# mbed92/soft-grip

Measured on AMD Instinct MI355X. Metric: env steps/sec (whole node) at batch=4096, higher is better.
Workload: dtype f64; 1 GPU; configs[2]: 4096 envs/GPU, softbox scene (nv=118), stiffness ~ U(300,1400), reference 200-step squeeze schedule from reset, 7 substeps per env step; 327 equality rows (composite neighbour equalities on: DESIGN.md 2, U2); volume tendon damper integrated explicitly; envs_per_gpu=4096, envs_flagged_bad=0

## Files before the change

### include/softgrip.h

```cpp
#ifndef SOFTGRIP_H
#define SOFTGRIP_H

#include <stddef.h>
#include <stdint.h>

#ifdef __cplusplus
extern "C" {
#endif

typedef struct sg_model sg_model;
typedef struct sg_batch sg_batch;

typedef enum sg_status {
  SG_OK = 0,
  SG_ERR_INVALID = -1,
  SG_ERR_MODEL = -2,
  SG_ERR_NO_DEVICE = -3,
  SG_ERR_HIP = -4,
  SG_ERR_NOMEM = -5
} sg_status;

enum {
  SG_FLAG_BADQPOS = 1, SG_FLAG_BADQVEL = 2, SG_FLAG_BADQACC = 4,
  SG_FLAG_CONTACTFULL = 8, SG_FLAG_CNSTRFULL = 16, SG_FLAG_UNSUPPORTED_PAIR = 32
// ... 37 lines not shown

int sg_get_state(sg_batch* b, double* qpos, double* qvel, double* act, double* qacc_warmstart, double* ctrl, void* stream);
int sg_set_state(sg_batch* b, const double* qpos, const double* qvel, const double* act, const double* qacc_warmstart,
                 const double* ctrl, void* stream);

int sg_get_solver_stats(sg_batch* b, int32_t* ncon, int32_t* nefc, int32_t* iters, void* stream);

int sg_set_pipeline(sg_batch* b, int pipeline);

int sg_get_touch_words(sg_batch* b, int32_t* out, int nwords, void* stream);
int sg_model_nboxes(const sg_model* m);

int sg_set_solver_envs_per_wavefront(sg_batch* b, int epw);
int sg_solver_envs_per_wavefront(const sg_batch* b);

int sg_tree_workgroups_per_cu(const sg_batch* b);

int sg_get_poses(sg_batch* b, const int32_t* env_ids, int n_ids, double* xpos, double* xquat, double* geom_xpos, double* geom_xmat, void* stream);
int sg_model_nbody(const sg_model* m);
int sg_model_ngeom(const sg_model* m);

int sg_model_default_camera(const sg_model* m, double cam[7]);
int sg_render(sg_batch* b, const double* cam, const int32_t* env_ids, int n_ids, int width, int height,
              uint8_t* rgba, float* depth, int32_t* segid, void* stream);

int sg_model_set_skin(sg_model* m, int nvert, const int32_t* vert_body, const double* vert_pos,
                      int nface, const int32_t* face, const float rgba[4]);
int sg_model_skin(const sg_model* m, int* nvert, int* nface, int32_t* vert_body, double* vert_pos,
                  int32_t* face, float* rgba);

// ... 17 lines not shown
```

### soft-grip_amd/build_native.py

```python
import concurrent.futures
import contextlib
import sys
import fcntl
import glob
import hashlib
import os
import shutil
import subprocess
import tempfile

_HERE = os.path.dirname(os.path.abspath(__file__))
if _HERE not in sys.path:
    sys.path.insert(0, _HERE)
CSRC = os.path.join(_HERE, "csrc")
LIB = os.path.join(_HERE, "libsoftgrip.so")
LEGACY_LIB = os.path.join(_HERE, "libsoftgrip_legacy.so")
SOURCES = ["sg_api.hip", "sg_phase.hip", "sg_rows.hip", "sg_tree.hip", "sg_plan.cpp", "sg_mjcf.cpp"]
LEGACY_SOURCES = ["sg_legacy.hip"]
FLAGS = ["--offload-arch=gfx950", "-O3", "-std=c++17", "-fPIC", "-mllvm", "-amdgpu-sched-strategy=iterative-ilp"]
SOURCE_FLAGS = {"sg_tree.hip": ["-fno-optimize-sibling-calls"]}


def _headers():
    return sorted(glob.glob(os.path.join(CSRC, "*.h")) + glob.glob(os.path.join(CSRC, "*.inc")) + glob.glob(os.path.join(_HERE, "..", "include", "*.h")) + [os.path.join(CSRC, "sg_kernels.hip"), os.path.join(CSRC, "sg_kin.hip"), os.path.join(CSRC, "sg_contacts.hip"), os.path.abspath(__file__)])


def _stale(target, deps):
    if not os.path.exists(target):
        return True
    t = os.path.getmtime(target)
    return any(os.path.getmtime(d) > t for d in deps)


def needs_build(lib=LIB, sources=SOURCES):
    return _stale(lib, [os.path.join(CSRC, s) for s in sources] + _headers())
# ... 128 lines not shown
```

### soft-grip_amd/csrc/sg_api.hip

```cpp
#include <hip/hip_runtime.h>

#include <cstdio>
#include <cstring>
#include <memory>
#include <string>
#include <vector>

#include "sg_mjcf.h"
#include "sg_tree.h"
#include "sg_work.h"
#include "sg_kin.hip"
#include "sg_contacts.hip"
#include "sg_devmem.h"
#ifdef SG_LEGACY_PIPELINES
#include "sg_kernels_args.h"
#endif

#ifdef SG_LEGACY_PIPELINES
#define SG_LEGACY_ON 1
#else
#define SG_LEGACY_ON 0
#endif

namespace {
// ... 56 lines not shown
struct sg_batch {
  const sg_model* m = nullptr;
  int n = 0, device = 0;
  SgArena mem;
  SgArena tree_mem;
  SgPlanHeader* dH = nullptr;
  double *delem = nullptr, *qpos = nullptr, *qvel = nullptr, *warm = nullptr, *act = nullptr, *ctrl = nullptr, *kenv = nullptr, *ctrl_row = nullptr;
  SgGenPair* dgpairs = nullptr;
  int* dnbtab = nullptr;
  SgEqSlot* dsched = nullptr;
  unsigned* dtab = nullptr;
  int* dcpos = nullptr;
  int *kmask_jnt = nullptr, *kmask_ten = nullptr, *flags = nullptr, *touch = nullptr, *ncon = nullptr, *nefc = nullptr, *iters = nullptr;
  std::vector<int> kmask_jnt_host, kmask_ten_host;
  int epw_override = 0;
  int pipeline = 3;
  SgTreeBufs t;
  bool tree_ready = false;
  bool tree_attr_set = false;
  SgWork w = {};
  bool lds_attr_set = false;
  bool prof = false;
  std::vector<std::pair<hipEvent_t, hipEvent_t>> ev;
  double prof_ms = 0;
  long long prof_n = 0;
  std::vector<std::pair<hipEvent_t, hipEvent_t>> ev_pgs;
  std::vector<hipEvent_t> ev_pool;
  double prof_pgs_ms = 0;
  long long prof_pgs_n = 0;
  double* kin_d = nullptr;
// ... 314 lines not shown
  list.clear();
  if (avg_ms) *avg_ms = count ? sum_ms / count : 0.0;
  if (launches) *launches = count;
  if (reset) { sum_ms = 0; count = 0; }
  return SG_OK;
}

#define SG_EPW8_MIN_WAVES 1024
static int solver_epw(const sg_batch* b) {
  if (b->m->plan.h.nnb > 0) return 4;
  if (b->epw_override) return b->epw_override;
  if (const char* pe = getenv("SG_PGS_EPW")) return atoi(pe) == 4 ? 4 : 8;
  return (b->n + 7) / 8 >= SG_EPW8_MIN_WAVES ? 8 : 4;
}

static int launch_split(sg_batch* b, int mode, const uint8_t* mask, int nsub, double* sens, long long stride, int32_t* flags, int32_t* touch,
                        hipStream_t s) {
  const SgPlanHeader& H = b->m->plan.h;
  SgPhaseArgs pa;
  pa.H = b->dH; pa.elem = b->delem;
  pa.qpos = b->qpos; pa.qvel = b->qvel; pa.warm = b->warm; pa.act = b->act; pa.ctrl = b->ctrl;
  pa.kenv = b->kenv; pa.kmask_jnt = b->kmask_jnt; pa.kmask_ten = b->kmask_ten;
  pa.mask = mask; pa.sens = nullptr; pa.sens_stride = stride > 0 ? stride : H.nsensordata;
  pa.w = b->w; pa.nenv = b->n; pa.rowlayout = b->pipeline == 2;
  pa.nbtab = b->dnbtab; pa.cpos = b->dcpos; pa.cst_rounds = (H.nnb > 0 && SG_ROWS_NB_MODE(H.nelem, H.eq_rounds) == 2) ? H.eq_rounds + 8 : 0;
  pa.gpairs = b->dgpairs;
  pa.nelem = H.nelem; pa.nv = H.nv; pa.nu = H.nu; pa.elem_dof0 = H.elem_dof0; pa.nchain = H.nchain; pa.t0_id = H.t0_id; pa.timestep = H.timestep;
  SgPgsArgs ga;
  ga.sched = b->dsched; ga.nbtab = b->dnbtab; ga.tab = b->dtab;
  ga.H = b->dH; ga.elem = b->delem; ga.w = b->w; ga.nenv = b->n;
  const size_t lds = sizeof(double) * ((size_t)(5 * 8 + 2) * H.nelem + 16 * 4 * SG_MAXLIM + 72);
  (void)lds;
  const int nsl = sg_rows_nsl(H.nelem);
  const bool nbm = H.nnb > 0;
  const int epw = solver_epw(b);
  const int nbmode = nbm ? SG_ROWS_NB_MODE(H.nelem, H.eq_rounds) : 0;
  const size_t lds_rows = sizeof(double) * (nbm ? SG_ROWS_LDS_NB(epw, H.nelem, H.eq_rounds, nbmode == 2) : SG_ROWS_LDS_FIX(epw, 8 * (size_t)nsl));
  if (!b->lds_attr_set) {
    HIPCHK(sg_rows_prepare());
#ifdef SG_LEGACY_PIPELINES
    HIPCHK(sg_legacy_prepare());
#endif
    b->lds_attr_set = true;
  }
  const int nfwd = nsub + (mode == 1 ? 1 : 0);
  size_t call_ev = 0;
  if (b->prof) {
    if (int rc = begin_event_pair(b, b->ev, s)) return rc;
    call_ev = b->ev.size() - 1;
  }
  const bool genpass = b->pipeline == 2;
  for (int k = 0; k <= nfwd; k++) {
    SgPhaseArgs p = pa;
    p.first = k == 0;
    p.do_reset = (mode == 1 && k == 0);
    p.do_finish = k > 0;
    p.finish_integrate = (mode == 1) ? (k > 1) : 1;
    p.do_begin = k < nfwd;
    p.sens = (k == nfwd) ? sens : nullptr;
    if (nfwd == 0) { p.do_begin = 0; p.do_finish = 0; }
    HIPCHK(sg_launch_chain(p, b->n, s));
    p.sens = nullptr;
    HIPCHK(sg_launch_phase(p, b->m->rounds, nbm, genpass, b->n, s));
    if (k < nfwd) {
      if (b->prof)
        if (int rc = begin_event_pair(b, b->ev_pgs, s)) return rc;
      if (b->pipeline == 2) HIPCHK(sg_launch_rows(ga, nsl, nbmode, epw, b->n, lds_rows, s));
#ifdef SG_LEGACY_PIPELINES
      else HIPCHK(sg_launch_pgs_split(ga, b->n, lds, s));
#endif
      if (b->prof) HIPCHK(hipEventRecord(b->ev_pgs.back().second, s));
    }
  }
  if (b->prof) HIPCHK(hipEventRecord(b->ev[call_ev].second, s));
  hipLaunchKernelGGL(sg_masked_copy_kernel, dim3((b->n + 255) / 256), dim3(256), 0, s, mask, b->n, b->w.status, flags ? flags : b->flags,
                     b->w.touch, touch ? touch : b->touch, b->w.ncon, b->ncon, b->w.nefc, b->nefc, b->w.iters, b->iters);
  HIPCHK(hipGetLastError());
  return SG_OK;
// ... 109 lines not shown
  if (!m) return 0;
  if (!m->has_fast) return m->tree.NG;
  int n = 0;
  for (int c = 0; c < m->plan.h.nchain; c++) n += m->plan.h.chain[c].ngeom;
  return n;
}

int sg_set_solver_envs_per_wavefront(sg_batch* b, int epw) {
  if (!b || (epw != 0 && epw != 4 && epw != 8)) return fail(SG_ERR_INVALID, "sg_set_solver_envs_per_wavefront: 0 (automatic), 4 or 8");
  if (b->m->plan.h.nnb > 0 && epw == 8)
    return fail(SG_ERR_MODEL, "sg_set_solver_envs_per_wavefront: a model with neighbour equality rows runs 4 envs of 16 lanes per wavefront");
  b->epw_override = epw;
  return SG_OK;
}
int sg_solver_envs_per_wavefront(const sg_batch* b) { return b ? solver_epw(b) : 0; }
int sg_tree_workgroups_per_cu(const sg_batch* b) {
  if (!b) return fail(SG_ERR_INVALID, "sg_tree_workgroups_per_cu: bad argument");
  if (!b->tree_ready) return 0;
  const sg_model* m = b->m;
  if (hipSetDevice(b->device) != hipSuccess) return fail(SG_ERR_NO_DEVICE, "hipSetDevice");
  if (sg_tree_prepare() != hipSuccess) return fail(SG_ERR_HIP, "sg_tree_prepare");
  return sg_tree_occupancy(m->tree.CS, m->tree_lds);
}

#ifdef SG_SECTION_PROF
int sg_debug_sections(sg_batch* b, unsigned long long* out32) {
  if (!b || !out32) return fail(SG_ERR_INVALID, "sg_debug_sections: bad argument");
  HIPCHK(hipSetDevice(b->device));
  HIPCHK(hipDeviceSynchronize());
  HIPCHK(hipMemcpy(out32, b->w.secprof, sizeof(unsigned long long) * 48, hipMemcpyDeviceToHost));
// ... 291 lines not shown
```

### soft-grip_amd/csrc/sg_phase.hip

```cpp
#include "sg_work.h"

struct GenLds {
  StageRec2* stage;
  double* gas;
  double* gg;
  double* tmp;
  const double (*boxp)[3];
  const double (*boxm)[9];
  const ChainKin* K;
  const ChainLds2* cs;
  const double *qe, *ve, *asme, *we;
};

__device__ __forceinline__ void sg_gen_capsule(const SgPhaseArgs& a, const GenLds& L, int e, double* cp, double* cax) {
  const int N = a.nelem;
  auto EL = [&](int f, int k) { return a.elem[(size_t)f * N + k]; };
  const double dq = L.qe[e] - EL(SGE_QPOS0, e);
  cp[0] = EL(SGE_GX, e) + EL(SGE_AX, e) * dq; cp[1] = EL(SGE_GY, e) + EL(SGE_AY, e) * dq; cp[2] = EL(SGE_GZ, e) + EL(SGE_AZ, e) * dq;
  cax[0] = EL(SGE_CX, e); cax[1] = EL(SGE_CY, e); cax[2] = EL(SGE_CZ, e);
}

__device__ __noinline__ int sg_gen_phase(const SgPhaseArgs& a, const SgPlanHeader& H, const int env, const GenLds L, int* flags, int* touch) {
  const int lane = threadIdx.x, N = a.nelem;
  auto EL = [&](int f, int k) { return a.elem[(size_t)f * N + k]; };
// ... 184 lines not shown
    gen_contact_load(c, rec);
    const double as_ = c.sl >= 0 ? as_lds[c.sl] : 0.0;
#pragma unroll
    for (int r = 0; r < 3; r++) {
      double Ja = c.Js[r] * as_;
#pragma unroll
      for (int ch = 0; ch < SG_MAXCH; ch++)
#pragma unroll
        for (int d = 0; d < SG_CD; d++) Ja += c.Jf[ch][r][d] * aF[ch][d];
      cp += c.f[r] * (0.5 * (Ja + c.R * c.f[r]) + c.b[r]);
    }
  }
  return cp;
}

template <int R, int CPL, bool NB, bool GEN>
__device__ __forceinline__ void sg_phase_env(const SgPhaseArgs& a, const int env) {
  const int lane = threadIdx.x;
  if (env >= a.nenv) return;
  if (a.mask && !a.mask[env]) return;
  SG_T0();
  const SG_CONSTAS SgPlanHeader& H = *(const SG_CONSTAS SgPlanHeader*)a.H;
  const int N = a.nelem, nv = a.nv, nu = a.nu, e0 = a.elem_dof0, nchain = a.nchain;
  const size_t S = 2 * (size_t)a.nenv;
  const double h = a.timestep;
  __shared__ Smem2<R, CPL, NB> Sm;
  const SG_CONSTAS double* const elemc = (const SG_CONSTAS double*)a.elem;
  [[maybe_unused]] const SG_CONSTAS int* const nbtabc = (const SG_CONSTAS int*)a.nbtab;
  auto EL = [&](int f, int e) { return elemc[(size_t)f * N + e]; };
  const int half = lane >> 5;
  const bool high = half != 0;
  const bool is_chain_lane = (lane & 31) == 0 && half < nchain;
  const SG_CONSTAS SgChain& C = H.chain[half < nchain ? half : 0];
  ChainLds2& CS = Sm.cs[half];
  const SgWork& W = a.w;
  [[maybe_unused]] unsigned short* const gpairs_env = W.gpairs16 + (size_t)env * SG_PAIRS_CAP(R);
  [[maybe_unused]] double* const gcval_env = W.gcval + (size_t)env * SG_MAXCH * (32 * CPL);
  auto pair_at = [&](int i) -> unsigned short& {
    if constexpr (SG_PHASE_SLIM(R)) return gpairs_env[i];
    else return Sm.pairs[i];
  };
  auto cval_at = [&](int cc, int i) -> double& {
    if constexpr (SG_PHASE_SLIM(R)) return gcval_env[cc * (32 * CPL) + i];
    else return Sm.cval[cc * (32 * CPL) + i];
  };

  int status = W.status[env];
  const int pend = W.pending[env];

  double* gq = a.qpos + (size_t)env * nv;
  double* gv = a.qvel + (size_t)env * nv;
  double* gw = a.warm + (size_t)env * nv;
  const double kenv = a.kenv[env];
  const int kt0_masked = a.kmask_ten[a.t0_id];

  double qe[R], ve[R], we[R], ke[R];
#pragma unroll
  for (int r = 0; r < R; r++) {
    int e = r * 64 + lane;
    qe[r] = ve[r] = we[r] = ke[r] = 0;
    if (e < N) {
      if (a.do_reset) { qe[r] = EL(SGE_QPOS0, e); }
      else { qe[r] = gq[e0 + e]; ve[r] = gv[e0 + e]; we[r] = gw[e0 + e]; }
      ke[r] = a.kmask_jnt[e0 + e] ? kenv : EL(SGE_K0, e);
    }
  }
  double ase[R], asme_p[R], fsm_p[R];
#pragma unroll
  for (int r = 0; r < R; r++) {
    const int e = r * 64 + lane;
    ase[r] = asme_p[r] = fsm_p[r] = 0;
    if (a.do_finish && e < N) {
      ase[r] = W.as[(size_t)env * N + e]; asme_p[r] = W.asme[(size_t)env * N + e];
      if (a.finish_integrate) fsm_p[r] = W.fsm[(size_t)env * N + e];
    }
  }
  if (a.do_begin && half < nchain) {
    const double* ch = W.chh + ((size_t)env * 2 + half) * SG_CHW;
    double* const kd = (double*)&Sm.K[half];
    double* const box = &Sm.boxp[half * SG_CG][0];
    double* const boxm = &Sm.boxm[half * SG_CG][0];
    double* const lim = CS.lim_sign;
#pragma unroll
    for (int j0 = 0; j0 < SG_CHW; j0 += 32) {
      const int j = j0 + (lane & 31);
      const double v = j < SG_CHW ? ch[j] : 0.0;
      if (j >= SGH_QSM && j < SGH_QSM + SG_CD) CS.qacc_smooth[j - SGH_QSM] = v;
      else if (j >= SGH_K && j < SGH_K + 48) kd[j - SGH_K] = v;
      else if (j >= SGH_MINV && j < SGH_MINV + 16) CS.Minv[j - SGH_MINV] = v;
      else if (j >= SGH_V && j < SGH_V + SG_CD) CS.v[j - SGH_V] = v;
      else if (j >= SGH_W && j < SGH_W + SG_CD) CS.w[j - SGH_W] = v;
      else if (j >= SGH_BOX && j < SGH_BOX + 12 * SG_CG) {
        const int g = (j - SGH_BOX) / 12, k = (j - SGH_BOX) % 12;
        if (k < 3) box[3 * g + k] = v; else boxm[9 * g + k - 3] = v;
      }
      else if (j == SGH_LIMACT) CS.lim_active = (int)v;
      else if (j >= SGH_LIMSIGN && j < SGH_LIMSIGN + 4 * SG_MAXLIM) lim[j - SGH_LIMSIGN] = v;
    }
  }
  const bool dead = (status & (SG_FLAG_BADQPOS | SG_FLAG_BADQVEL | SG_FLAG_BADQACC)) != 0;
  if (dead) return;
  const bool fin = a.do_finish && pend;
  const double kt0 = kt0_masked ? kenv : H.t0_k0;
  __syncthreads();

  SG_T(0);
  if (fin) {
    int badacc = 0;
    double qacc_e[R];
#pragma unroll
    for (int r = 0; r < R; r++) {
      int e = r * 64 + lane;
      qacc_e[r] = 0;
      if (e < N) {
// ... 632 lines not shown
    if (e < N) { gq[e0 + e] = qe[r]; gv[e0 + e] = ve[r]; gw[e0 + e] = we[r]; }
  }
  if (lane == 0) {
    if (status | flags) atomicOr(&W.status[env], status | flags);
  }
  SG_T(9);
  SG_TEND();
}

#ifndef SG_X_PHASE_OCC
#define SG_X_PHASE_OCC 2
#endif
#ifndef SG_X_CPL
#define SG_X_CPL 2
#endif
template <int R, int CPL, bool NB, bool GEN = false>
__global__ __launch_bounds__(64, SG_X_PHASE_OCC) void sg_phase_kernel(SgPhaseArgs a) {
  if constexpr (GEN) {
    const int cnt = a.w.gen_count[0];
    a.do_finish = 0; a.do_reset = 0; a.sens = nullptr;
    for (int i = blockIdx.x; i < cnt && i < a.nenv; i += gridDim.x) {
      sg_phase_env<R, CPL, NB, true>(a, a.w.gen_list[i]);
      __syncthreads();
    }
  } else {
    sg_phase_env<R, CPL, NB, false>(a, blockIdx.x);
  }
}

__global__ __launch_bounds__(64) void sg_chain_kernel(SgPhaseArgs a) {
  const int lane = threadIdx.x, c = blockIdx.x & 1, env = (int)(blockIdx.x >> 1) * 64 + lane;
  if (blockIdx.x == 0 && lane == 0) a.w.gen_count[0] = 0;
  SG_T0();
  const SG_CONSTAS SgPlanHeader& H = *(const SG_CONSTAS SgPlanHeader*)a.H;
  const int nv = a.nv, nu = a.nu;
  const size_t S = 2 * (size_t)a.nenv;
  if (env >= a.nenv) return;
  const size_t st = 2 * (size_t)env + c;
  if (a.mask && !a.mask[env]) return;
  SgWork& W = a.w;
  if (a.first && c == 0) { W.status[env] = 0; if (!a.do_finish) W.pending[env] = 0; }
  if (c >= a.nchain) return;
  const int status = a.first ? 0 : W.status[env];
  const int pend = a.do_finish ? W.pending[env] : 0;
  const SgChain& C = H.chain[c];
  const double h = a.timestep;
  double* gq = a.qpos + (size_t)env * nv;
  double* gv = a.qvel + (size_t)env * nv;
  double* gw = a.warm + (size_t)env * nv;
  const double kenv = a.kenv[env];
  double q[SG_CD], v[SG_CD], w[SG_CD], kk[SG_CD], act = 0, ctrl = 0;
#pragma unroll
  for (int d = 0; d < SG_CD; d++) {
    int j = C.dof0 + d;
    if (a.do_reset) { q[d] = C.qpos0[d]; v[d] = 0; w[d] = 0; }
    else { q[d] = gq[j]; v[d] = gv[j]; w[d] = gw[j]; }
    kk[d] = a.kmask_jnt[j] ? kenv : C.stiffness[d];
  }
  if (C.has_act) {
    if (a.do_reset) a.ctrl[(size_t)env * nu + C.act_id] = 0;
    else { act = a.act[(size_t)env * nu + C.act_id]; ctrl = a.ctrl[(size_t)env * nu + C.act_id]; }
  }
  const double kten = C.has_ten ? (a.kmask_ten[C.ten_id] ? kenv : C.ten_k0) : 0.0;
  double* ch = W.chh + st * SG_CHW;
  bool bad_acc = false;
  if (status & (SG_FLAG_BADQPOS | SG_FLAG_BADQVEL | SG_FLAG_BADQACC)) return;

  SG_T(17);
  if (a.do_finish && pend) {
    double aF[SG_CD], qacc_c[SG_CD];
#pragma unroll
    for (int d = 0; d < SG_CD; d++) {
      aF[d] = W.saF[(size_t)d * S + st];
      qacc_c[d] = ch[SGH_QSM + d] + aF[d];
      if (isbad(qacc_c[d])) bad_acc = true;
    }
    ChainKin K;
    {
      double* kd = (double*)&K;
#pragma unroll
      for (int i = 0; i < 48; i++) kd[i] = ch[SGH_K + i];
    }
    if (a.sens) {
      ChainMotion Mo;
// ... 50 lines not shown
            for (int b2 = 0; b2 < SG_CD; b2++) s2 += MhBinv[4 * a2 + b2] * rhs[b2];
            qa[a2] = s2;
          }
        } else {
#pragma unroll
          for (int d = 0; d < SG_CD; d++) qa[d] = qacc_c[d];
        }
        act += h * ch[SGH_ACTDOT];
#pragma unroll
        for (int d = 0; d < SG_CD; d++) { v[d] += h * qa[d]; q[d] += h * v[d]; }
      }
    }
  }

  SG_T(18);
  if (a.do_begin && !bad_acc) {
    int bad = 0;
#pragma unroll
    for (int d = 0; d < SG_CD; d++) bad |= (isbad(q[d]) ? SG_FLAG_BADQPOS : 0) | (isbad(v[d]) ? SG_FLAG_BADQVEL : 0);
    if (bad) {
      atomicOr(&W.status[env], bad);
    } else {
      ChainKin K;
      ChainDyn D;
      chain_kinematics(C, q, K);
      SG_T(19);
      chain_dynamics(C, K, q, v, act, ctrl, kk, kten, H.gravity, D);
      SG_T(20);
      double rec[SG_CHW];
#pragma unroll
      for (int i = 0; i < SG_CHW; i++) rec[i] = 0.0;
// ... 18 lines not shown
          mulmat33(bm2, bm_, C.g_mat[g]);
        }
#pragma unroll
        for (int k = 0; k < 3; k++) rec[SGH_BOX + 12 * g + k] = bp_[k] + t[k];
#pragma unroll
        for (int k = 0; k < 9; k++) rec[SGH_BOX + 12 * g + 3 + k] = bm2[k];
      }
      SG_T(21);
      LimitRows L;
      limits_build(C, q, v, D.qacc_smooth, w, L);
      rec[SGH_LIMACT] = (double)L.active;
#pragma unroll
      for (int k = 0; k < SG_MAXLIM; k++) { rec[SGH_LIMSIGN + k] = L.sign[k]; rec[SGH_LIMR + k] = L.R[k]; rec[SGH_LIMB + k] = L.b[k]; rec[SGH_LIMF + k] = L.f[k]; }
      static_assert(SG_CHW % 2 == 0 && SGH_LIMF + SG_MAXLIM <= SG_CHW, "hand-off record layout");
#pragma unroll
      for (int i = 0; i < (SGH_LIMF + SG_MAXLIM + 1) / 2; i++) ((double2*)ch)[i] = make_double2(rec[2 * i], rec[2 * i + 1]);
    }
  }
  SG_T(22);
#pragma unroll
  for (int d = 0; d < SG_CD; d++) { int j = C.dof0 + d; gq[j] = q[d]; gv[j] = v[d]; gw[j] = w[d]; }
  if (C.has_act) a.act[(size_t)env * nu + C.act_id] = act;
  SG_T(23);
  SG_TEND();
}


hipError_t sg_launch_chain(const SgPhaseArgs& p, int nenv, hipStream_t s) {
  hipLaunchKernelGGL(sg_chain_kernel, dim3(2 * ((nenv + 63) / 64)), dim3(64), 0, s, p);
  return hipGetLastError();
}
hipError_t sg_launch_phase(const SgPhaseArgs& p, int rounds, bool nb, bool genpass, int nenv, hipStream_t s) {
#define SG_PHASE(r)                                                                                   \
  if (nb) {                                                                                           \
    hipLaunchKernelGGL((sg_phase_kernel<r, SG_X_CPL, true>), dim3(nenv), dim3(64), 0, s, p);                 \
    if (genpass && p.do_begin) hipLaunchKernelGGL((sg_phase_kernel<r, 2, true, true>), dim3(nenv < SG_GEN_GRID ? nenv : SG_GEN_GRID), dim3(64), 0, s, p); \
  } else {                                                                                            \
    hipLaunchKernelGGL((sg_phase_kernel<r, SG_X_CPL, false>), dim3(nenv), dim3(64), 0, s, p);                \
    if (genpass && p.do_begin) hipLaunchKernelGGL((sg_phase_kernel<r, 2, false, true>), dim3(nenv < SG_GEN_GRID ? nenv : SG_GEN_GRID), dim3(64), 0, s, p); \
  }
  switch (rounds) {
    case 1: SG_PHASE(1); break;
    case 2: SG_PHASE(2); break;
    case 3: SG_PHASE(3); break;
    default: SG_PHASE(4); break;
  }
#undef SG_PHASE
  return hipGetLastError();
}
```

### soft-grip_amd/csrc/sg_work.h

```cpp
#pragma once
#include <hip/hip_runtime.h>

#include "../../include/softgrip.h"
#include "sg_math.h"
#include "sg_general.h"

using namespace sgm;

#define SG_CAP 64
#define SG_NF 26
#define SG_RF 30
#define SG_REC_INDEX(slot, wave, field, pos, nwb) (((((size_t)(slot)) * ((nwb) + 1) + (wave)) * SG_RF + (field)) * SG_SPW + (pos))
#define SG_G 8
#define SG_EPW (64 / SG_G)
#define SG_SPW (2 * SG_EPW)
#define SG_GEN_GRID 256
#define SG_CHW 160

struct SgWork {
  double* crec;
  unsigned long long* secprof;
  double* crow;
  double* cdummy;
  int* ns;
// ... 110 lines not shown

struct SgPgsArgs {
  const unsigned* tab;
  const SgEqSlot* sched;
  const int* nbtab;
  const SgPlanHeader* H;
  const double* elem;
  SgWork w;
  int nenv;
};

#define SG_ROWS_LDS_FIX(EPW, NR) ((size_t)(5 * (EPW) + 2) * (NR) + 72)
#define SG_ROWS_NA_NB(N) (((N) + 2) & ~1)
#define SG_ROWS_LDS_NB(EPW, N, ROUNDS, CST) ((size_t)(EPW) * SG_ROWS_NA_NB(N) + (size_t)((CST) ? 4 : 8) * (EPW) * ((N) + 1) + (size_t)((CST) ? 8 : 16) * ((ROUNDS) + 8) + 72 + 2 * (EPW))
#define SG_ROWS_NB_MODE(N, ROUNDS) (sizeof(double) * SG_ROWS_LDS_NB(4, N, ROUNDS, 0) <= 40 * 1024 ? 1 : 2)
hipError_t sg_launch_chain(const SgPhaseArgs& p, int nenv, hipStream_t s);
hipError_t sg_launch_phase(const SgPhaseArgs& p, int rounds, bool nb, bool genpass, int nenv, hipStream_t s);
hipError_t sg_rows_prepare();
int sg_rows_nsl(int nelem);
hipError_t sg_launch_rows(const SgPgsArgs& a, int nsl, int nb , int epw, int nenv, size_t lds_bytes, hipStream_t s);
#ifdef SG_LEGACY_PIPELINES
struct SgKArgs;
hipError_t sg_legacy_prepare();
hipError_t sg_launch_pgs_split(const SgPgsArgs& a, int nenv, size_t lds_bytes, hipStream_t s);
hipError_t sg_launch_fused(const SgKArgs& a, int rounds, int nenv, hipStream_t s);
#endif
```

### soft-grip_amd/native.py

```python
import ctypes as C
import os

import numpy as np

_HERE = os.path.dirname(os.path.abspath(__file__))
LIB_PATH = os.path.join(_HERE, "libsoftgrip.so")
_LIB = None

SG_OK, SG_ERR_INVALID, SG_ERR_MODEL, SG_ERR_NO_DEVICE, SG_ERR_HIP, SG_ERR_NOMEM = 0, -1, -2, -3, -4, -5
SG_FLAG_BADQPOS, SG_FLAG_BADQVEL, SG_FLAG_BADQACC, SG_FLAG_CONTACTFULL, SG_FLAG_CNSTRFULL, SG_FLAG_UNSUPPORTED_PAIR = 1, 2, 4, 8, 16, 32
FLAG_BADQPOS, FLAG_BADQVEL, FLAG_BADQACC, FLAG_CONTACTFULL, FLAG_CNSTRFULL, FLAG_UNSUPPORTED_PAIR = 1, 2, 4, 8, 16, 32

SYMBOLS = [
    "sg_last_error", "sg_version", "sg_model_create", "sg_model_destroy", "sg_model_nq", "sg_model_nu",
    "sg_model_nsensordata", "sg_model_ntendon", "sg_model_nelem", "sg_batch_create", "sg_batch_destroy",
    "sg_batch_nenvs", "sg_batch_device", "sg_set_stiffness", "sg_set_ctrl", "sg_reset", "sg_step", "sg_get_state",
    "sg_set_state", "sg_get_solver_stats", "sg_set_pipeline", "sg_profile_enable", "sg_profile_read", "sg_profile_read_solver",
    "sg_model_compile", "sg_mjcf_compile", "sg_blob_free", "sg_set_solver_envs_per_wavefront", "sg_solver_envs_per_wavefront",
    "sg_get_touch_words", "sg_model_nboxes", "sg_model_nv", "sg_model_njnt", "sg_tree_workgroups_per_cu",
    "sg_get_poses", "sg_model_nbody", "sg_model_ngeom", "sg_model_default_camera", "sg_render",
    "sg_get_contacts", "sg_model_ncollision_pairs", "sg_model_set_skin", "sg_model_skin", "sg_render_ex",
]
SG_RENDER_SKIN = 1
SG_COMPILE_NO_NEIGHBORS, SG_COMPILE_IMPLICIT_TENDON_DAMPER = 1, 2


class SoftgripError(RuntimeError):
    def __init__(self, code, msg):
        super().__init__("softgrip error %d: %s" % (code, msg))
        self.code = code


def lib():
    global _LIB
    if _LIB is None:
        if not os.path.exists(LIB_PATH):
# ... 23 lines not shown
    L.sg_batch_create.argtypes = [vp, C.c_int, C.c_int, C.POINTER(vp)]
    L.sg_batch_destroy.argtypes = [vp]
    L.sg_batch_destroy.restype = None
    L.sg_batch_nenvs.argtypes = [vp]
    L.sg_batch_device.argtypes = [vp]
    L.sg_set_stiffness.argtypes = [vp, vp, C.c_int, C.POINTER(C.c_int), C.c_int, C.POINTER(C.c_int), C.c_int, vp]
    L.sg_set_ctrl.argtypes = [vp, vp, C.c_int, vp]
    L.sg_reset.argtypes = [vp, vp, C.c_int, dp, ip, ip, vp]
    L.sg_step.argtypes = [vp, C.c_int, dp, i64, ip, ip, vp]
    L.sg_get_state.argtypes = [vp, dp, dp, dp, dp, dp, vp]
    L.sg_set_state.argtypes = [vp, dp, dp, dp, dp, dp, vp]
    L.sg_get_solver_stats.argtypes = [vp, ip, ip, ip, vp]
    L.sg_set_pipeline.argtypes = [vp, C.c_int]
    L.sg_set_solver_envs_per_wavefront.argtypes = [vp, C.c_int]
    L.sg_solver_envs_per_wavefront.argtypes = [vp]
    L.sg_tree_workgroups_per_cu.argtypes = [vp]
    L.sg_model_nbody.argtypes = [vp]
    L.sg_model_ngeom.argtypes = [vp]
    L.sg_model_default_camera.argtypes = [vp, C.POINTER(C.c_double)]
    L.sg_get_poses.argtypes = [vp, C.POINTER(C.c_int32), C.c_int, dp, dp, dp, dp, vp]
    L.sg_render.argtypes = [vp, C.POINTER(C.c_double), C.POINTER(C.c_int32), C.c_int, C.c_int, C.c_int, vp, vp, vp, vp]
    L.sg_model_set_skin.argtypes = [vp, C.c_int, ip, dp, C.c_int, ip, C.POINTER(C.c_float)]
    L.sg_model_skin.argtypes = [vp, C.POINTER(C.c_int), C.POINTER(C.c_int), ip, dp, ip, C.POINTER(C.c_float)]
    L.sg_render_ex.argtypes = [vp, C.POINTER(C.c_double), C.POINTER(C.c_int32), C.c_int, C.c_int, C.c_int, C.c_int, vp, vp, vp, vp]
    L.sg_get_contacts.argtypes = [vp, C.POINTER(C.c_int32), C.c_int, C.c_int, ip, ip, dp, dp, dp, vp]
    L.sg_model_ncollision_pairs.argtypes = [vp]
    L.sg_profile_enable.argtypes = [vp, C.c_int]
    L.sg_profile_read.argtypes = [vp, C.c_int, C.POINTER(C.c_double), C.POINTER(C.c_longlong)]
    L.sg_profile_read_solver.argtypes = [vp, C.c_int, C.POINTER(C.c_double), C.POINTER(C.c_longlong)]
    return L
# ... 207 lines not shown
        args = (_ptr(out.get("rgba")), _ptr(out.get("depth")), _ptr(out.get("seg")), self._stream())
        head = (self.ptr, cam.ctypes.data_as(C.POINTER(C.c_double)), None if ids is None else ids.ctypes.data_as(C.POINTER(C.c_int32)), k,
                int(width), int(height))
        if skin:
            self._check(self.L.sg_render_ex(*head, SG_RENDER_SKIN, *args))
        else:
            self._check(self.L.sg_render(*head, *args))
        return out

    def set_solver_envs_per_wavefront(self, epw):
        self._check(self.L.sg_set_solver_envs_per_wavefront(self.ptr, int(epw)))

    def solver_envs_per_wavefront(self):
        return self.L.sg_solver_envs_per_wavefront(self.ptr)

    def tree_workgroups_per_cu(self):
        return self.L.sg_tree_workgroups_per_cu(self.ptr)

    def profile_enable(self, on=True):
        self._check(self.L.sg_profile_enable(self.ptr, int(on)))

    def profile_read(self, reset=True):
        ms, n = C.c_double(), C.c_longlong()
        self._check(self.L.sg_profile_read(self.ptr, int(reset), C.byref(ms), C.byref(n)))
        return ms.value, n.value

    def profile_read_solver(self, reset=True):
        ms, n = C.c_double(), C.c_longlong()
        self._check(self.L.sg_profile_read_solver(self.ptr, int(reset), C.byref(ms), C.byref(n)))
        return ms.value, n.value
# ... 1 lines not shown
```

Measured before the change: 1.116 million env-steps/s.

## Make phase kernel persistent with next-env prefetch and stage chain records through LDS

```diff
diff --git a/include/softgrip.h b/include/softgrip.h
--- a/include/softgrip.h
+++ b/include/softgrip.h
@@ -75,6 +75,9 @@
 int sg_set_solver_envs_per_wavefront(sg_batch* b, int epw);
 int sg_solver_envs_per_wavefront(const sg_batch* b);
 
+int sg_set_phase_wavefronts(sg_batch* b, int n);
+int sg_phase_wavefronts(sg_batch* b);
+
 int sg_tree_workgroups_per_cu(const sg_batch* b);
 
 int sg_get_poses(sg_batch* b, const int32_t* env_ids, int n_ids, double* xpos, double* xquat, double* geom_xpos, double* geom_xmat, void* stream);
diff --git a/soft-grip_amd/build_native.py b/soft-grip_amd/build_native.py
--- a/soft-grip_amd/build_native.py
+++ b/soft-grip_amd/build_native.py
@@ -18,7 +18,7 @@
 SOURCES = ["sg_api.hip", "sg_phase.hip", "sg_rows.hip", "sg_tree.hip", "sg_plan.cpp", "sg_mjcf.cpp"]
 LEGACY_SOURCES = ["sg_legacy.hip"]
 FLAGS = ["--offload-arch=gfx950", "-O3", "-std=c++17", "-fPIC", "-mllvm", "-amdgpu-sched-strategy=iterative-ilp"]
-SOURCE_FLAGS = {"sg_tree.hip": ["-fno-optimize-sibling-calls"]}
+SOURCE_FLAGS = {"sg_tree.hip": ["-fno-optimize-sibling-calls"], "sg_phase.hip": ["-mllvm", "-disable-machine-licm"]}
 
 
 def _headers():
diff --git a/soft-grip_amd/csrc/sg_api.hip b/soft-grip_amd/csrc/sg_api.hip
--- a/soft-grip_amd/csrc/sg_api.hip
+++ b/soft-grip_amd/csrc/sg_api.hip
@@ -94,6 +94,8 @@
   int *kmask_jnt = nullptr, *kmask_ten = nullptr, *flags = nullptr, *touch = nullptr, *ncon = nullptr, *nefc = nullptr, *iters = nullptr;
   std::vector<int> kmask_jnt_host, kmask_ten_host;
   int epw_override = 0;
+  int phase_waves_override = 0;
+  int phase_resident = 0;
   int pipeline = 3;
   SgTreeBufs t;
   bool tree_ready = false;
@@ -438,6 +440,13 @@
   return (b->n + 7) / 8 >= SG_EPW8_MIN_WAVES ? 8 : 4;
 }
 
+static int phase_grid(sg_batch* b, int* grid) {
+  if (b->phase_waves_override) { *grid = b->phase_waves_override < b->n ? b->phase_waves_override : b->n; return SG_OK; }
+  if (!b->phase_resident) HIPCHK(sg_phase_resident(b->m->rounds, b->m->plan.h.nnb > 0, &b->phase_resident));
+  *grid = b->phase_resident < b->n ? b->phase_resident : b->n;
+  return SG_OK;
+}
+
 static int launch_split(sg_batch* b, int mode, const uint8_t* mask, int nsub, double* sens, long long stride, int32_t* flags, int32_t* touch,
                         hipStream_t s) {
   const SgPlanHeader& H = b->m->plan.h;
@@ -462,12 +471,15 @@
   const size_t lds_rows = sizeof(double) * (nbm ? SG_ROWS_LDS_NB(epw, H.nelem, H.eq_rounds, nbmode == 2) : SG_ROWS_LDS_FIX(epw, 8 * (size_t)nsl));
   if (!b->lds_attr_set) {
     HIPCHK(sg_rows_prepare());
+    HIPCHK(sg_phase_prepare());
 #ifdef SG_LEGACY_PIPELINES
     HIPCHK(sg_legacy_prepare());
 #endif
     b->lds_attr_set = true;
   }
   const int nfwd = nsub + (mode == 1 ? 1 : 0);
+  int pgrid = 0;
+  if (int rc = phase_grid(b, &pgrid)) return rc;
   size_t call_ev = 0;
   if (b->prof) {
     if (int rc = begin_event_pair(b, b->ev, s)) return rc;
@@ -485,7 +497,7 @@
     if (nfwd == 0) { p.do_begin = 0; p.do_finish = 0; }
     HIPCHK(sg_launch_chain(p, b->n, s));
     p.sens = nullptr;
-    HIPCHK(sg_launch_phase(p, b->m->rounds, nbm, genpass, b->n, s));
+    HIPCHK(sg_launch_phase(p, b->m->rounds, nbm, genpass, b->n, pgrid, s));
     if (k < nfwd) {
       if (b->prof)
         if (int rc = begin_event_pair(b, b->ev_pgs, s)) return rc;
@@ -625,6 +637,20 @@
   return SG_OK;
 }
 int sg_solver_envs_per_wavefront(const sg_batch* b) { return b ? solver_epw(b) : 0; }
+int sg_set_phase_wavefronts(sg_batch* b, int n) {
+  if (!b || n < 0) return fail(SG_ERR_INVALID, "sg_set_phase_wavefronts: 0 (automatic) or a number of wavefronts");
+  if (!b->m->has_fast) return fail(SG_ERR_MODEL, "sg_set_phase_wavefronts: the model is outside the two-finger class, the tree pipeline has no phase kernel");
+  b->phase_waves_override = n;
+  return SG_OK;
+}
+int sg_phase_wavefronts(sg_batch* b) {
+  if (!b) return fail(SG_ERR_INVALID, "sg_phase_wavefronts: bad argument");
+  if (!b->m->has_fast) return 0;
+  HIPCHK(hipSetDevice(b->device));
+  int grid = 0;
+  if (int rc = phase_grid(b, &grid)) return rc;
+  return grid;
+}
 int sg_tree_workgroups_per_cu(const sg_batch* b) {
   if (!b) return fail(SG_ERR_INVALID, "sg_tree_workgroups_per_cu: bad argument");
   if (!b->tree_ready) return 0;
diff --git a/soft-grip_amd/csrc/sg_phase.hip b/soft-grip_amd/csrc/sg_phase.hip
--- a/soft-grip_amd/csrc/sg_phase.hip
+++ b/soft-grip_amd/csrc/sg_phase.hip
@@ -222,19 +222,72 @@
   return cp;
 }
 
-template <int R, int CPL, bool NB, bool GEN>
-__device__ __forceinline__ void sg_phase_env(const SgPhaseArgs& a, const int env) {
-  const int lane = threadIdx.x;
-  if (env >= a.nenv) return;
-  if (a.mask && !a.mask[env]) return;
+template <int R>
+struct SgPhasePre {
+  int status, pend;
+  double kenv;
+  double qe[R], ve[R], we[R];
+  double ase[R], asme[R], fsm[R];
+  double ch[SG_CHW / 32];
+};
+
+template <int R>
+__device__ __forceinline__ void sg_phase_prefetch(const SgPhaseArgs& a, const int env, const int lane, SgPhasePre<R>& P) {
+  static_assert(SG_CHW % 32 == 0, "the 32 lanes of a half import the hand-off record in whole rounds");
+  const int N = a.nelem, nv = a.nv, e0 = a.elem_dof0, half = lane >> 5;
+  const SgWork& W = a.w;
+  P.status = W.status[env];
+  P.pend = W.pending[env];
+  P.kenv = ((const SG_CONSTAS double*)a.kenv)[env];
+  const double* gq = a.qpos + (size_t)env * nv;
+  const double* gv = a.qvel + (size_t)env * nv;
+  const double* gw = a.warm + (size_t)env * nv;
+#pragma unroll
+  for (int r = 0; r < R; r++) {
+    const int e = r * 64 + lane;
+    P.qe[r] = P.ve[r] = P.we[r] = 0;
+    if (e < N && !a.do_reset) { P.qe[r] = gq[e0 + e]; P.ve[r] = gv[e0 + e]; P.we[r] = gw[e0 + e]; }
+  }
+#pragma unroll
+  for (int r = 0; r < R; r++) {
+    const int e = r * 64 + lane;
+    P.ase[r] = P.asme[r] = P.fsm[r] = 0;
+    if (a.do_finish && e < N) {
+      P.ase[r] = W.as[(size_t)env * N + e]; P.asme[r] = W.asme[(size_t)env * N + e];
+      if (a.finish_integrate) P.fsm[r] = W.fsm[(size_t)env * N + e];
+    }
+  }
+#pragma unroll
+  for (int k = 0; k < SG_CHW / 32; k++) P.ch[k] = 0.0;
+  if (a.do_begin && half < a.nchain) {
+    const double* ch = W.chh + ((size_t)env * 2 + half) * SG_CHW;
+#pragma unroll
+    for (int k = 0; k < SG_CHW / 32; k++) P.ch[k] = ch[32 * k + (lane & 31)];
+  }
+}
+
+template <int R, int CPL, bool NB, bool GEN, bool WALK>
+__device__ __forceinline__ void sg_phase_env(const SgPhaseArgs& a, const int env, const int lane, SgPhasePre<R>& P, const int next) {
   SG_T0();
-  const SG_CONSTAS SgPlanHeader& H = *(const SG_CONSTAS SgPlanHeader*)a.H;
+  const SgPlanHeader* Hp = a.H;
+  const double* elemp = a.elem;
+  const int *nbtabp = a.nbtab, *kmjp = a.kmask_jnt;
+#if SG_X_PHASE_LAUNDER & 2
+  if constexpr (WALK) {
+    int z = 0;
+    asm volatile("" : "+v"(z));
+    z = __builtin_amdgcn_readfirstlane(z);
+    Hp = (const SgPlanHeader*)((const char*)Hp + z); elemp = (const double*)((const char*)elemp + z);
+    nbtabp = (const int*)((const char*)nbtabp + z); kmjp = (const int*)((const char*)kmjp + z);
+  }
+#endif
+  const SG_CONSTAS SgPlanHeader& H = *(const SG_CONSTAS SgPlanHeader*)Hp;
   const int N = a.nelem, nv = a.nv, nu = a.nu, e0 = a.elem_dof0, nchain = a.nchain;
   const size_t S = 2 * (size_t)a.nenv;
   const double h = a.timestep;
   __shared__ Smem2<R, CPL, NB> Sm;
-  const SG_CONSTAS double* const elemc = (const SG_CONSTAS double*)a.elem;
-  [[maybe_unused]] const SG_CONSTAS int* const nbtabc = (const SG_CONSTAS int*)a.nbtab;
+  const SG_CONSTAS double* const elemc = (const SG_CONSTAS double*)elemp;
+  [[maybe_unused]] const SG_CONSTAS int* const nbtabc = (const SG_CONSTAS int*)nbtabp;
   auto EL = [&](int f, int e) { return elemc[(size_t)f * N + e]; };
   const int half = lane >> 5;
   const bool high = half != 0;
@@ -253,38 +306,29 @@
     else return Sm.cval[cc * (32 * CPL) + i];
   };
 
-  int status = W.status[env];
-  const int pend = W.pending[env];
+  int status = P.status;
+  const int pend = P.pend;
 
   double* gq = a.qpos + (size_t)env * nv;
   double* gv = a.qvel + (size_t)env * nv;
   double* gw = a.warm + (size_t)env * nv;
-  const double kenv = a.kenv[env];
+  const double kenv = P.kenv;
   const int kt0_masked = a.kmask_ten[a.t0_id];
 
   double qe[R], ve[R], we[R], ke[R];
 #pragma unroll
   for (int r = 0; r < R; r++) {
     int e = r * 64 + lane;
-    qe[r] = ve[r] = we[r] = ke[r] = 0;
+    qe[r] = P.qe[r]; ve[r] = P.ve[r]; we[r] = P.we[r]; ke[r] = 0;
     if (e < N) {
       if (a.do_reset) { qe[r] = EL(SGE_QPOS0, e); }
-      else { qe[r] = gq[e0 + e]; ve[r] = gv[e0 + e]; we[r] = gw[e0 + e]; }
-      ke[r] = a.kmask_jnt[e0 + e] ? kenv : EL(SGE_K0, e);
+      ke[r] = kmjp[e0 + e] ? kenv : EL(SGE_K0, e);
     }
   }
   double ase[R], asme_p[R], fsm_p[R];
 #pragma unroll
-  for (int r = 0; r < R; r++) {
-    const int e = r * 64 + lane;
-    ase[r] = asme_p[r] = fsm_p[r] = 0;
-    if (a.do_finish && e < N) {
-      ase[r] = W.as[(size_t)env * N + e]; asme_p[r] = W.asme[(size_t)env * N + e];
-      if (a.finish_integrate) fsm_p[r] = W.fsm[(size_t)env * N + e];
-    }
-  }
+  for (int r = 0; r < R; r++) { ase[r] = P.ase[r]; asme_p[r] = P.asme[r]; fsm_p[r] = P.fsm[r]; }
   if (a.do_begin && half < nchain) {
-    const double* ch = W.chh + ((size_t)env * 2 + half) * SG_CHW;
     double* const kd = (double*)&Sm.K[half];
     double* const box = &Sm.boxp[half * SG_CG][0];
     double* const boxm = &Sm.boxm[half * SG_CG][0];
@@ -292,7 +336,7 @@
 #pragma unroll
     for (int j0 = 0; j0 < SG_CHW; j0 += 32) {
       const int j = j0 + (lane & 31);
-      const double v = j < SG_CHW ? ch[j] : 0.0;
+      const double v = P.ch[j0 / 32];
       if (j >= SGH_QSM && j < SGH_QSM + SG_CD) CS.qacc_smooth[j - SGH_QSM] = v;
       else if (j >= SGH_K && j < SGH_K + 48) kd[j - SGH_K] = v;
       else if (j >= SGH_MINV && j < SGH_MINV + 16) CS.Minv[j - SGH_MINV] = v;
@@ -306,6 +350,7 @@
       else if (j >= SGH_LIMSIGN && j < SGH_LIMSIGN + 4 * SG_MAXLIM) lim[j - SGH_LIMSIGN] = v;
     }
   }
+  if (next >= 0) sg_phase_prefetch<R>(a, next, lane, P);
   const bool dead = (status & (SG_FLAG_BADQPOS | SG_FLAG_BADQVEL | SG_FLAG_BADQACC)) != 0;
   if (dead) return;
   const bool fin = a.do_finish && pend;
@@ -968,60 +1013,125 @@
 #ifndef SG_X_CPL
 #define SG_X_CPL 2
 #endif
-template <int R, int CPL, bool NB, bool GEN = false>
+#ifndef SG_X_PHASE_LAUNDER
+#define SG_X_PHASE_LAUNDER 3
+#endif
+#ifndef SG_PHASE_AHEAD
+#define SG_PHASE_AHEAD(R) ((R) <= 2)
+#endif
+#define SG_PHASE_WALKS(R) ((R) <= 2)
+template <int R, int CPL, bool NB, bool GEN = false, bool WALK = true>
 __global__ __launch_bounds__(64, SG_X_PHASE_OCC) void sg_phase_kernel(SgPhaseArgs a) {
   if constexpr (GEN) {
     const int cnt = a.w.gen_count[0];
     a.do_finish = 0; a.do_reset = 0; a.sens = nullptr;
     for (int i = blockIdx.x; i < cnt && i < a.nenv; i += gridDim.x) {
-      sg_phase_env<R, CPL, NB, true>(a, a.w.gen_list[i]);
+      const int env = a.w.gen_list[i];
+      SgPhasePre<R> P;
+      sg_phase_prefetch<R>(a, env, threadIdx.x, P);
+      sg_phase_env<R, CPL, NB, true, false>(a, env, threadIdx.x, P, -1);
       __syncthreads();
     }
+  } else if constexpr (!WALK) {
+    const int env = blockIdx.x;
+    if (env < a.nenv && (!a.mask || a.mask[env])) {
+      SgPhasePre<R> P;
+      sg_phase_prefetch<R>(a, env, threadIdx.x, P);
+      sg_phase_env<R, CPL, NB, false, false>(a, env, threadIdx.x, P, -1);
+    }
   } else {
-    sg_phase_env<R, CPL, NB, false>(a, blockIdx.x);
+    const int nenv = a.nenv, grid = gridDim.x;
+    const unsigned char* const mask = a.mask;
+    int env = blockIdx.x;
+    bool have = env < nenv && (!mask || mask[env]);
+    SgPhasePre<R> P;
+    if (have) sg_phase_prefetch<R>(a, env, threadIdx.x, P);
+    while (env < nenv) {
+      int lane = threadIdx.x;
+#if SG_X_PHASE_LAUNDER & 1
+      asm volatile("" : "+v"(lane));
+      __builtin_assume(lane >= 0 && lane < 64);
+#endif
+      const int next = env + grid;
+      const bool nhave = next < nenv && (!mask || mask[next]);
+      if (have) {
+        if constexpr (SG_PHASE_AHEAD(R)) {
+          sg_phase_env<R, CPL, NB, false, true>(a, env, lane, P, nhave ? next : -1);
+          __syncthreads();
+        } else {
+          sg_phase_env<R, CPL, NB, false, true>(a, env, lane, P, -1);
+          __syncthreads();
+          if (nhave) sg_phase_prefetch<R>(a, next, lane, P);
+        }
+      } else if (nhave) {
+        sg_phase_prefetch<R>(a, next, lane, P);
+      }
+      env = next; have = nhave;
+    }
   }
 }
 
+#define SG_CHT (SG_CHW + 2)
+#define SG_CHAIN_LDS (64 * SG_CHT * sizeof(double))
 __global__ __launch_bounds__(64) void sg_chain_kernel(SgPhaseArgs a) {
-  const int lane = threadIdx.x, c = blockIdx.x & 1, env = (int)(blockIdx.x >> 1) * 64 + lane;
+  extern __shared__ double sg_chain_tile[];
+  const int lane = threadIdx.x, c = blockIdx.x & 1, env0 = (int)(blockIdx.x >> 1) * 64, env = env0 + lane;
   if (blockIdx.x == 0 && lane == 0) a.w.gen_count[0] = 0;
   SG_T0();
   const SG_CONSTAS SgPlanHeader& H = *(const SG_CONSTAS SgPlanHeader*)a.H;
   const int nv = a.nv, nu = a.nu;
   const size_t S = 2 * (size_t)a.nenv;
-  if (env >= a.nenv) return;
+  const bool live = env < a.nenv && (!a.mask || a.mask[env]);
   const size_t st = 2 * (size_t)env + c;
-  if (a.mask && !a.mask[env]) return;
   SgWork& W = a.w;
-  if (a.first && c == 0) { W.status[env] = 0; if (!a.do_finish) W.pending[env] = 0; }
+  if (live && a.first && c == 0) { W.status[env] = 0; if (!a.do_finish) W.pending[env] = 0; }
   if (c >= a.nchain) return;
-  const int status = a.first ? 0 : W.status[env];
-  const int pend = a.do_finish ? W.pending[env] : 0;
+  constexpr int FIN_UNITS = (SGH_K + 48 + 1) / 2, REC_UNITS = SG_CHW / 2;
+  static_assert(SGH_QSM + SG_CD <= 2 * FIN_UNITS && SGH_QFRC + SG_CD <= 2 * FIN_UNITS && SGH_ACTDOT < 2 * FIN_UNITS &&
+                SGH_M + 16 <= 2 * FIN_UNITS && 2 * FIN_UNITS <= SG_CHW, "what FINISH reads of the hand-off record");
+  if (a.do_finish) {
+    const int nu16 = (a.nenv - env0 < 64 ? a.nenv - env0 : 64) * FIN_UNITS;
+    double2 t[FIN_UNITS];
+#pragma unroll
+    for (int it = 0; it < FIN_UNITS; it++) {
+      const int u = it * 64 + lane, r = u / FIN_UNITS, k = u - r * FIN_UNITS;
+      t[it] = make_double2(0.0, 0.0);
+      if (u < nu16) t[it] = *(const double2*)(W.chh + (2 * (size_t)(env0 + r) + c) * SG_CHW + 2 * k);
+    }
+#pragma unroll
+    for (int it = 0; it < FIN_UNITS; it++) {
+      const int u = it * 64 + lane, r = u / FIN_UNITS, k = u - r * FIN_UNITS;
+      *(double2*)(sg_chain_tile + r * SG_CHT + 2 * k) = t[it];
+    }
+  }
+  const int status = live && !a.first ? W.status[env] : 0;
+  const int pend = live && a.do_finish ? W.pending[env] : 0;
   const SgChain& C = H.chain[c];
   const double h = a.timestep;
   double* gq = a.qpos + (size_t)env * nv;
   double* gv = a.qvel + (size_t)env * nv;
   double* gw = a.warm + (size_t)env * nv;
-  const double kenv = a.kenv[env];
+  const double kenv = live ? a.kenv[env] : 0.0;
   double q[SG_CD], v[SG_CD], w[SG_CD], kk[SG_CD], act = 0, ctrl = 0;
 #pragma unroll
   for (int d = 0; d < SG_CD; d++) {
     int j = C.dof0 + d;
-    if (a.do_reset) { q[d] = C.qpos0[d]; v[d] = 0; w[d] = 0; }
+    if (a.do_reset || !live) { q[d] = C.qpos0[d]; v[d] = 0; w[d] = 0; }
     else { q[d] = gq[j]; v[d] = gv[j]; w[d] = gw[j]; }
     kk[d] = a.kmask_jnt[j] ? kenv : C.stiffness[d];
   }
-  if (C.has_act) {
+  if (C.has_act && live) {
     if (a.do_reset) a.ctrl[(size_t)env * nu + C.act_id] = 0;
     else { act = a.act[(size_t)env * nu + C.act_id]; ctrl = a.ctrl[(size_t)env * nu + C.act_id]; }
   }
   const double kten = C.has_ten ? (a.kmask_ten[C.ten_id] ? kenv : C.ten_k0) : 0.0;
-  double* ch = W.chh + st * SG_CHW;
+  double* const ch = sg_chain_tile + lane * SG_CHT;
   bool bad_acc = false;
-  if (status & (SG_FLAG_BADQPOS | SG_FLAG_BADQVEL | SG_FLAG_BADQACC)) return;
+  const bool run = live && !(status & (SG_FLAG_BADQPOS | SG_FLAG_BADQVEL | SG_FLAG_BADQACC));
+  __syncthreads();
 
   SG_T(17);
-  if (a.do_finish && pend) {
+  if (run && a.do_finish && pend) {
     double aF[SG_CD], qacc_c[SG_CD];
 #pragma unroll
     for (int d = 0; d < SG_CD; d++) {
@@ -1102,7 +1212,9 @@
   }
 
   SG_T(18);
-  if (a.do_begin && !bad_acc) {
+  __syncthreads();
+  bool wrote = false;
+  if (run && a.do_begin && !bad_acc) {
     int bad = 0;
 #pragma unroll
     for (int d = 0; d < SG_CD; d++) bad |= (isbad(q[d]) ? SG_FLAG_BADQPOS : 0) | (isbad(v[d]) ? SG_FLAG_BADQVEL : 0);
@@ -1151,29 +1263,74 @@
       for (int k = 0; k < SG_MAXLIM; k++) { rec[SGH_LIMSIGN + k] = L.sign[k]; rec[SGH_LIMR + k] = L.R[k]; rec[SGH_LIMB + k] = L.b[k]; rec[SGH_LIMF + k] = L.f[k]; }
       static_assert(SG_CHW % 2 == 0 && SGH_LIMF + SG_MAXLIM <= SG_CHW, "hand-off record layout");
 #pragma unroll
-      for (int i = 0; i < (SGH_LIMF + SG_MAXLIM + 1) / 2; i++) ((double2*)ch)[i] = make_double2(rec[2 * i], rec[2 * i + 1]);
+      for (int i = 0; i < REC_UNITS; i++) ((double2*)ch)[i] = make_double2(rec[2 * i], rec[2 * i + 1]);
+      wrote = true;
+    }
+  }
+  __syncthreads();
+  const unsigned long long wrote_m = __ballot(wrote);
+  if (wrote_m) {
+#pragma unroll 8
+    for (int it = 0; it < REC_UNITS; it++) {
+      const int u = it * 64 + lane, r = u / REC_UNITS, k = u - r * REC_UNITS;
+      if ((wrote_m >> r) & 1ull) *(double2*)(W.chh + (2 * (size_t)(env0 + r) + c) * SG_CHW + 2 * k) = *(const double2*)(sg_chain_tile + r * SG_CHT + 2 * k);
     }
   }
   SG_T(22);
-#pragma unroll
-  for (int d = 0; d < SG_CD; d++) { int j = C.dof0 + d; gq[j] = q[d]; gv[j] = v[d]; gw[j] = w[d]; }
-  if (C.has_act) a.act[(size_t)env * nu + C.act_id] = act;
+  if (run) {
+#pragma unroll
+    for (int d = 0; d < SG_CD; d++) { int j = C.dof0 + d; gq[j] = q[d]; gv[j] = v[d]; gw[j] = w[d]; }
+    if (C.has_act) a.act[(size_t)env * nu + C.act_id] = act;
+  }
   SG_T(23);
   SG_TEND();
 }
 
 
+hipError_t sg_phase_prepare() {
+  return hipFuncSetAttribute((const void*)sg_chain_kernel, hipFuncAttributeMaxDynamicSharedMemorySize, (int)SG_CHAIN_LDS);
+}
 hipError_t sg_launch_chain(const SgPhaseArgs& p, int nenv, hipStream_t s) {
-  hipLaunchKernelGGL(sg_chain_kernel, dim3(2 * ((nenv + 63) / 64)), dim3(64), 0, s, p);
+  hipLaunchKernelGGL(sg_chain_kernel, dim3(2 * ((nenv + 63) / 64)), dim3(64), SG_CHAIN_LDS, s, p);
   return hipGetLastError();
 }
-hipError_t sg_launch_phase(const SgPhaseArgs& p, int rounds, bool nb, bool genpass, int nenv, hipStream_t s) {
+hipError_t sg_phase_resident(int rounds, bool nb, int* out) {
+  if (!SG_PHASE_WALKS(rounds < 4 ? rounds : 4)) { *out = 0x7fffffff; return hipSuccess; }
+  int dev = 0, cus = 0, per_cu = 0;
+  hipError_t e = hipGetDevice(&dev);
+  if (e == hipSuccess) e = hipDeviceGetAttribute(&cus, hipDeviceAttributeMultiprocessorCount, dev);
+#define SG_PHASE_OCC(r)                                                                                                                    \
+  if (e == hipSuccess) e = nb ? hipOccupancyMaxActiveBlocksPerMultiprocessor(&per_cu, sg_phase_kernel<r, SG_X_CPL, true>, 64, 0)          \
+                              : hipOccupancyMaxActiveBlocksPerMultiprocessor(&per_cu, sg_phase_kernel<r, SG_X_CPL, false>, 64, 0)
+  switch (rounds) {
+    case 1: SG_PHASE_OCC(1); break;
+    case 2: SG_PHASE_OCC(2); break;
+    case 3: SG_PHASE_OCC(3); break;
+    default: SG_PHASE_OCC(4); break;
+  }
+#undef SG_PHASE_OCC
+  if (e == hipSuccess && (per_cu < 1 || cus < 1)) e = hipErrorInvalidValue;
+  if (e == hipSuccess) *out = per_cu * cus;
+  return e;
+}
+template <int R, bool NB>
+static void sg_launch_phase_main(const SgPhaseArgs& p, int nenv, int grid, hipStream_t s) {
+  if constexpr (!SG_PHASE_WALKS(R)) {
+    if (grid == nenv) {
+      hipLaunchKernelGGL((sg_phase_kernel<R, SG_X_CPL, NB, false, false>), dim3(nenv), dim3(64), 0, s, p);
+      return;
+    }
+  }
+  hipLaunchKernelGGL((sg_phase_kernel<R, SG_X_CPL, NB>), dim3(grid), dim3(64), 0, s, p);
+}
+hipError_t sg_launch_phase(const SgPhaseArgs& p, int rounds, bool nb, bool genpass, int nenv, int grid, hipStream_t s) {
+  if (grid < 1 || grid > nenv) return hipErrorInvalidValue;
 #define SG_PHASE(r)                                                                                   \
   if (nb) {                                                                                           \
-    hipLaunchKernelGGL((sg_phase_kernel<r, SG_X_CPL, true>), dim3(nenv), dim3(64), 0, s, p);                 \
+    sg_launch_phase_main<r, true>(p, nenv, grid, s);                                                  \
     if (genpass && p.do_begin) hipLaunchKernelGGL((sg_phase_kernel<r, 2, true, true>), dim3(nenv < SG_GEN_GRID ? nenv : SG_GEN_GRID), dim3(64), 0, s, p); \
   } else {                                                                                            \
-    hipLaunchKernelGGL((sg_phase_kernel<r, SG_X_CPL, false>), dim3(nenv), dim3(64), 0, s, p);                \
+    sg_launch_phase_main<r, false>(p, nenv, grid, s);                                                 \
     if (genpass && p.do_begin) hipLaunchKernelGGL((sg_phase_kernel<r, 2, false, true>), dim3(nenv < SG_GEN_GRID ? nenv : SG_GEN_GRID), dim3(64), 0, s, p); \
   }
   switch (rounds) {
diff --git a/soft-grip_amd/csrc/sg_work.h b/soft-grip_amd/csrc/sg_work.h
--- a/soft-grip_amd/csrc/sg_work.h
+++ b/soft-grip_amd/csrc/sg_work.h
@@ -148,8 +148,10 @@
 #define SG_ROWS_NA_NB(N) (((N) + 2) & ~1)
 #define SG_ROWS_LDS_NB(EPW, N, ROUNDS, CST) ((size_t)(EPW) * SG_ROWS_NA_NB(N) + (size_t)((CST) ? 4 : 8) * (EPW) * ((N) + 1) + (size_t)((CST) ? 8 : 16) * ((ROUNDS) + 8) + 72 + 2 * (EPW))
 #define SG_ROWS_NB_MODE(N, ROUNDS) (sizeof(double) * SG_ROWS_LDS_NB(4, N, ROUNDS, 0) <= 40 * 1024 ? 1 : 2)
+hipError_t sg_phase_prepare();
 hipError_t sg_launch_chain(const SgPhaseArgs& p, int nenv, hipStream_t s);
-hipError_t sg_launch_phase(const SgPhaseArgs& p, int rounds, bool nb, bool genpass, int nenv, hipStream_t s);
+hipError_t sg_launch_phase(const SgPhaseArgs& p, int rounds, bool nb, bool genpass, int nenv, int grid, hipStream_t s);
+hipError_t sg_phase_resident(int rounds, bool nb, int* out);
 hipError_t sg_rows_prepare();
 int sg_rows_nsl(int nelem);
 hipError_t sg_launch_rows(const SgPgsArgs& a, int nsl, int nb , int epw, int nenv, size_t lds_bytes, hipStream_t s);
diff --git a/soft-grip_amd/native.py b/soft-grip_amd/native.py
--- a/soft-grip_amd/native.py
+++ b/soft-grip_amd/native.py
@@ -20,6 +20,7 @@
     "sg_get_touch_words", "sg_model_nboxes", "sg_model_nv", "sg_model_njnt", "sg_tree_workgroups_per_cu",
     "sg_get_poses", "sg_model_nbody", "sg_model_ngeom", "sg_model_default_camera", "sg_render",
     "sg_get_contacts", "sg_model_ncollision_pairs", "sg_model_set_skin", "sg_model_skin", "sg_render_ex",
+    "sg_set_phase_wavefronts", "sg_phase_wavefronts",
 ]
 SG_RENDER_SKIN = 1
 SG_COMPILE_NO_NEIGHBORS, SG_COMPILE_IMPLICIT_TENDON_DAMPER = 1, 2
@@ -73,6 +74,9 @@
     L.sg_set_pipeline.argtypes = [vp, C.c_int]
     L.sg_set_solver_envs_per_wavefront.argtypes = [vp, C.c_int]
     L.sg_solver_envs_per_wavefront.argtypes = [vp]
+    if hasattr(L, "sg_set_phase_wavefronts"):
+        L.sg_set_phase_wavefronts.argtypes = [vp, C.c_int]
+        L.sg_phase_wavefronts.argtypes = [vp]
     L.sg_tree_workgroups_per_cu.argtypes = [vp]
     L.sg_model_nbody.argtypes = [vp]
     L.sg_model_ngeom.argtypes = [vp]
@@ -310,6 +314,15 @@
     def solver_envs_per_wavefront(self):
         return self.L.sg_solver_envs_per_wavefront(self.ptr)
 
+    def set_phase_wavefronts(self, n):
+        self._check(self.L.sg_set_phase_wavefronts(self.ptr, int(n)))
+
+    def phase_wavefronts(self):
+        n = self.L.sg_phase_wavefronts(self.ptr)
+        if n < 0:
+            self._check(n)
+        return n
+
     def tree_workgroups_per_cu(self):
         return self.L.sg_tree_workgroups_per_cu(self.ptr)
 
```

Result: no change. 1.105 million env-steps/s (-1.0%).
